# acerbilab/gpyreg

Measured on AMD Instinct MI355X. Metric: GP-fits/sec (NLL+grad, N=4096 D=10), higher is better.
Workload: dtype f64

## Files before the change

### gpyreg_amd/csrc/blas1.h

```cpp
#pragma once
#include "common.h"

namespace gpc {

template <typename T>
__global__ __launch_bounds__(256) void trmv_kernel(const T* __restrict__ W_all, long long sW, int ldw,
                                                   const double* __restrict__ r_all, int npad,
                                                   double* __restrict__ z_all, int row0) {
  using vec_t = typename MM<T>::vec_t;
  constexpr int VEC = MM<T>::VEC;
  const int b = blockIdx.y, lane = threadIdx.x & 63;
  const int i = row0 + blockIdx.x * 4 + (threadIdx.x >> 6);
  const T* Wr = W_all + (size_t)b * sW + (size_t)i * ldw;
  const double* r = r_all + (size_t)b * npad;
  const int kend = ((i >> 7) + 1) << 7;
  double s = 0.0;
  for (int k = row0 + lane * VEC; k < kend; k += 64 * VEC) {
    const vec_t wv = *reinterpret_cast<const vec_t*>(Wr + k);
#pragma unroll
    for (int e = 0; e < VEC; ++e) s += (double)wv[e] * r[k + e];
  }
  s = wave_sum(s);
  if (lane == 0) z_all[(size_t)b * npad + i] = s;
}
// ... 129 lines not shown
  __shared__ double red[4][64 * MM<T>::VEC];
  trmv_t_part_body<T, UNR>(W_all, sW, ldw, z_all, npad, part_all, quad, red);
}
template <typename T>
__global__ __launch_bounds__(256) void trmv_t_part_low_kernel(
    const T* __restrict__ W_all, long long sW, int ldw, const double* __restrict__ z_all, int npad,
    double* __restrict__ part_all, double* __restrict__ quad) {
  __shared__ double red[4][64 * MM<T>::VEC];
  __builtin_amdgcn_s_setprio(3);
  trmv_t_part_body<T, 3>(W_all, sW, ldw, z_all, npad, part_all, quad, red);
}

__global__ __launch_bounds__(128) void trmv_t_sum_kernel(const double* __restrict__ part_all, int npad,
                                                         const double* __restrict__ sp_all, int sp_stride,
                                                         int sp_off, double* __restrict__ out_all) {
  const int b = blockIdx.y, k = blockIdx.x * 128 + threadIdx.x;
  const int nch = npad / TRC;
  double v = 0.0;
  for (int ch = k / TRC; ch < nch; ++ch) v += part_all[((size_t)b * nch + ch) * npad + k];
  if (sp_all) v /= sp_all[(size_t)b * sp_stride + sp_off];
  out_all[(size_t)b * npad + k] = v;
}

__global__ __launch_bounds__(256) void dot_kernel(const double* __restrict__ x, const double* __restrict__ y,
                                                  int n, int stride, double* __restrict__ out) {
  __shared__ double sh4[4];
  const int b = blockIdx.y;
  double s = 0.0;
  for (int i = threadIdx.x; i < n; i += 256) s += x[(size_t)b * stride + i] * y[(size_t)b * stride + i];
  s = block_sum_256(s, sh4);
  if (threadIdx.x == 0) out[b] = s;
}

__global__ __launch_bounds__(256) void mat_t_vec_kernel(const double* __restrict__ Mat, int n, int P,
                                                        const double* __restrict__ vec, int vstride,
                                                        double* __restrict__ out) {
  __shared__ double sh4[4];
  const int p = blockIdx.x, b = blockIdx.y;
  double s = 0.0;
  for (int i = threadIdx.x; i < n; i += 256)
    s += Mat[((size_t)b * n + i) * P + p] * vec[(size_t)b * vstride + i];
  s = block_sum_256(s, sh4);
  if (threadIdx.x == 0) out[(size_t)b * P + p] = s;
}

__global__ __launch_bounds__(256) void grad_tail_kernel(const double* __restrict__ part, int ntiles, int P,
// ... 290 lines not shown
```

### gpyreg_amd/csrc/gemm.h

```cpp
#pragma once
#include "common.h"

#include <type_traits>

namespace gpc {

template <typename T>
constexpr int BKT_v = sizeof(T) == 4 ? 32 : 16;
template <typename T>
constexpr bool MM_SWZ = sizeof(T) == 4;
template <typename T>
constexpr int LDQ_v = MM_SWZ<T> ? BKT_v<T> : BKT_v<T> + 1;
constexpr int ldp_of(int BT) { return BT + 16; }
template <typename T>
constexpr int opsz_of(int BT) {
  return BKT_v<T> * (BT + 16) > BT * LDQ_v<T> ? BKT_v<T> * (BT + 16) : BT * LDQ_v<T>;
}

enum { KLO_ZERO = 0, KLO_ROW = 1, KLO_COL = 2 };
enum { KHI_FULL = 0, KHI_ROW = 1, KHI_COL = 2 };

struct GemmArgs {
  const void* A;
  const void* B;
  void* C;
  long long sA, sB, sC;
  int lda, ldb, ldc;
  int M, N, K;
  double alpha;
  int beta;
  int klo, khi, lower_only;
  int tiles_m, tiles_n;
  int flags = 0;
  const unsigned short* rsv = nullptr;
  int* ctr = nullptr;
  int ntiles = 0, batch = 0;
  double* colsq = nullptr;
  const double* ep_w = nullptr;
  long long ep_sw = 0;
  const double* ep_alpha = nullptr;
};
inline int g_gemm_flags = 8 | 16;

template <typename T, bool KM, int BT, int NT>
__device__ __forceinline__ unsigned stage_toff(int ld, int t) {
  constexpr int VEC = MM<T>::VEC;
  if constexpr (!KM) {
    constexpr int TPR = BKT_v<T> / VEC;
    return (unsigned)(t / TPR) * (unsigned)ld + (unsigned)((t % TPR) * VEC);
  } else {
    constexpr int VPR = BT / VEC;
    return (unsigned)(t / VPR) * (unsigned)ld + (unsigned)((t % VPR) * VEC);
  }
}
template <typename T, bool KM, int BT, int NT>
__device__ __forceinline__ size_t stage_pstride(int ld) {
  constexpr int VEC = MM<T>::VEC;
  if constexpr (!KM)
    return (size_t)(NT / (BKT_v<T> / VEC)) * ld;
  else
    return (size_t)(NT / (BT / VEC)) * ld;
}
template <typename T, bool KM, int BT, int NT, int AUX = 0>
// ... 47 lines not shown

template <typename T, bool KM, int BT>
__device__ __forceinline__ T frag(const T* __restrict__ s, int r0, int kk, int lane) {
  if constexpr (!KM) {
    if constexpr (MM_SWZ<T>) {
      constexpr int VEC = MM<T>::VEC;
      const int k = kk + (lane >> 4), l15 = lane & 15;
      return s[(r0 + l15) * LDQ_v<T> + (((k / VEC) ^ ((l15 >> 1) & 7)) * VEC) + (k % VEC)];
    } else {
      return s[(r0 + (lane & 15)) * LDQ_v<T> + kk + (lane >> 4)];
    }
  }
  else
    return s[(kk + (lane >> 4)) * ldp_of(BT) + r0 + (lane & 15)];
}

__device__ __forceinline__ void tri_tile(int tile, int& ti, int& tj) {
  int i = (int)((sqrtf(8.f * (float)tile + 1.f) - 1.f) * 0.5f);
  while (i * (i + 1) / 2 > tile) --i;
  while ((i + 1) * (i + 2) / 2 <= tile) ++i;
  ti = i;
  tj = tile - i * (i + 1) / 2;
}

#ifdef GPC_TILE_TRACE
__device__ unsigned long long g_tile_trace[2][4];
#define TILE_TS(k) do { if (HO && threadIdx.x == 0) { const long long _n = wall_clock64(); atomicAdd(&g_tile_trace[BT == 64][k], (unsigned long long)(_n - _ts)); _ts = _n; } } while (0)
#else
#define TILE_TS(k) do { } while (0)
#endif
template <typename T, bool AKM, bool BKM, int BT, int NW, int HO = 0, int EPI = 0, int BTN = BT>
__device__ __forceinline__ void gemm_tile(const GemmArgs& g, const int bx, const int by, T* __restrict__ smem) {
#ifdef GPC_TILE_TRACE
  long long _ts = wall_clock64();
  if (HO && threadIdx.x == 0) atomicAdd(&g_tile_trace[BT == 64][3], 1ull);
#endif
  using acc_t = typename MM<T>::acc_t;
  using vec_t = typename MM<T>::vec_t;
  constexpr int NT = 64 * NW;
  constexpr int NVA = (BT * BKT_v<T>) / (NT * MM<T>::VEC), NVB = (BTN * BKT_v<T>) / (NT * MM<T>::VEC);
  constexpr int OPSZA = opsz_of<T>(BT), OPSZB = opsz_of<T>(BTN), STG = OPSZA + OPSZB;
  constexpr int WCOLS = NW / 2;
  constexpr int WTM = BT / 2;
  constexpr int WTN = BTN / WCOLS;
  constexpr int MRM = WTM / 16, MRN = WTN / 16;
  static_assert(NVA >= 1 && NVB >= 1 && MRM >= 1 && MRN >= 1, "tile shape");
// ... 30 lines not shown
  int k0 = g.klo == KLO_ROW ? m128 : (g.klo == KLO_COL ? n128 : 0);
  int k1 = g.khi == KHI_ROW ? m128 + TILE : (g.khi == KHI_COL ? n128 + TILE : g.K);
  if (k1 > g.K) k1 = g.K;
  const int nk = (k1 - k0) / BKT_v<T>;

  const T* __restrict__ A = reinterpret_cast<const T*>(g.A) + (size_t)by * g.sA;
  const T* __restrict__ B = reinterpret_cast<const T*>(g.B) + (size_t)by * g.sB;
  T* __restrict__ C = reinterpret_cast<T*>(g.C) + (size_t)by * g.sC;

  acc_t acc[MRM][MRN];
#pragma unroll
  for (int i = 0; i < MRM; ++i)
#pragma unroll
    for (int j = 0; j < MRN; ++j) acc[i][j] = acc_t{0, 0, 0, 0};
  constexpr bool TWO_LEVEL = sizeof(T) == 4;
  acc_t acc2[TWO_LEVEL ? MRM : 1][TWO_LEVEL ? MRN : 1];
  if constexpr (TWO_LEVEL) {
#pragma unroll
    for (int i = 0; i < MRM; ++i)
#pragma unroll
      for (int j = 0; j < MRN; ++j) acc2[i][j] = acc_t{0, 0, 0, 0};
  }

  if (nk > 0) {
    vec_t ra[NVA], rb[NVB];
    const unsigned toa = stage_toff<T, AKM, BT, NT>(g.lda, t) * (unsigned)sizeof(T),
                   tob = stage_toff<T, BKM, BTN, NT>(g.ldb, t) * (unsigned)sizeof(T);
    const unsigned psa = (unsigned)(stage_pstride<T, AKM, BT, NT>(g.lda) * sizeof(T)),
                   psb = (unsigned)(stage_pstride<T, BKM, BTN, NT>(g.ldb) * sizeof(T));
    const T* pa = AKM ? A + (size_t)k0 * g.lda + m0 : A + (size_t)m0 * g.lda + k0;
    const T* pb = BKM ? B + (size_t)k0 * g.ldb + n0 : B + (size_t)n0 * g.ldb + k0;
    const size_t rowsa = (size_t)BKT_v<T> * g.lda, rowsb = (size_t)BKT_v<T> * g.ldb;
    __amdgpu_buffer_rsrc_t rsa = make_rsrc(pa), rsb = make_rsrc(pb);
    unsigned ua = 0, ub = 0;
    auto next_slab = [&]() {
      if constexpr (AKM) {
        pa += rowsa;
        rsa = make_rsrc(pa);
      } else {
        ua += (unsigned)(BKT_v<T> * sizeof(T));
      }
      if constexpr (BKM) {
        pb += rowsb;
        rsb = make_rsrc(pb);
      } else {
        ub += (unsigned)(BKT_v<T> * sizeof(T));
      }
    };
    constexpr int AUX = HO == 1 ? 16 : 0;
    g2r<T, AKM, BT, NT, AUX>(ra, rsa, ua, psa, toa);
    g2r<T, BKM, BTN, NT, AUX>(rb, rsb, ub, psb, tob);
    r2s<T, AKM, BT, NT>(smem, ra, t);
    r2s<T, BKM, BTN, NT>(smem + OPSZA, rb, t);
    next_slab();
    g2r<T, AKM, BT, NT, AUX>(ra, rsa, ua, psa, toa);
    g2r<T, BKM, BTN, NT, AUX>(rb, rsb, ub, psb, tob);
    __syncthreads();
    TILE_TS(0);

    T af[2][MRM], bf[2][MRN];
    auto load_frags = [&](int set, const T* a_s, const T* b_s, int kk) {
#pragma unroll
      for (int i = 0; i < MRM; ++i) af[set][i] = frag<T, AKM, BT>(a_s, wr * WTM + i * 16, kk, lane);
#pragma unroll
      for (int j = 0; j < MRN; ++j) bf[set][j] = frag<T, BKM, BTN>(b_s, wc * WTN + j * 16, kk, lane);
    };
    auto mfmas = [&](int set) {
#pragma unroll
      for (int i = 0; i < MRM; ++i)
#pragma unroll
        for (int j = 0; j < MRN; ++j) acc[i][j] = MM<T>::mma(af[set][i], bf[set][j], acc[i][j]);
    };
    constexpr int NMEM = NVA + NVB;
    constexpr int PER = (MRM * MRN) / NMEM;
    constexpr int REM = MRM * MRN - PER * NMEM;
    static_assert(PER >= 1, "interleave pattern");
    constexpr int KS = BKT_v<T> / 4;
    static_assert(KS >= 4 && KS % 2 == 0, "fragment sets alternate per k-step and wrap per slab");
    auto slab = [&](auto cur_c, auto wr_c, auto ld_c) {
// ... 124 lines not shown
          else
            v = al * acc[i][j][r];
          v += old[j][r];
          const double d = (double)v;
          cs[j] = fma(wr4[r] * d, d, cs[j]);
        }
    }
#pragma unroll
    for (int j = 0; j < MRN; ++j) {
      cs[j] += __shfl_xor(cs[j], 16, 64);
      cs[j] += __shfl_xor(cs[j], 32, 64);
    }
    double* red = reinterpret_cast<double*>(smem);
    __syncthreads();
    if ((lane >> 4) == 0) {
#pragma unroll
      for (int j = 0; j < MRN; ++j) red[wr * BT + wc * WTN + j * 16 + (lane & 15)] = cs[j];
    }
    __syncthreads();
    if (t < BT) g.colsq[((size_t)by * g.tiles_m + ti) * (size_t)g.N + n0 + t] = red[t] + red[BT + t];
    __syncthreads();
    return;
  }
#pragma unroll
  for (int i = 0; i < MRM; ++i) {
    T old[MRN][4];
    if (g.beta) {
#pragma unroll
      for (int j = 0; j < MRN; ++j)
#pragma unroll
        for (int r = 0; r < 4; ++r) {
          const int row = m0 + wr * WTM + i * 16 + MM<T>::row_of(lane, r);
          const int col = n0 + wc * WTN + j * 16 + (lane & 15);
          if constexpr (HO == 1)
            old[j][r] = __hip_atomic_load(&C[(size_t)row * g.ldc + col], __ATOMIC_RELAXED, __HIP_MEMORY_SCOPE_AGENT);
          else
            old[j][r] = C[(size_t)row * g.ldc + col];
        }
    }
#pragma unroll
    for (int j = 0; j < MRN; ++j)
#pragma unroll
      for (int r = 0; r < 4; ++r) {
        const int row = m0 + wr * WTM + i * 16 + MM<T>::row_of(lane, r);
        const int col = n0 + wc * WTN + j * 16 + (lane & 15);
        T v;
        if constexpr (TWO_LEVEL)
          v = alpha * (acc[i][j][r] + acc2[i][j][r]);
        else
          v = alpha * acc[i][j][r];
        if (g.beta) v += old[j][r];
        if constexpr (HO)
          __hip_atomic_store(&C[(size_t)row * g.ldc + col], v, __ATOMIC_RELAXED, __HIP_MEMORY_SCOPE_AGENT);
        else
          C[(size_t)row * g.ldc + col] = v;
      }
  }
  TILE_TS(2);
}

template <typename T, bool AKM, bool BKM, int BT, int NW, int EPI = 0, int BTN = BT>
__global__ __launch_bounds__(64 * NW, NW / 2) void gemm_kernel(GemmArgs g) {
  __shared__ __attribute__((aligned(16))) T smem[2 * (opsz_of<T>(BT) + opsz_of<T>(BTN))];
  int bx = blockIdx.x, by = blockIdx.y;
  if ((g.flags & 16) && gridDim.y >= 8) {
    const int total = gridDim.x * gridDim.y, per = total >> 3;
    const int L = blockIdx.y * gridDim.x + blockIdx.x;
    if (L < (per << 3)) {
      const int wk = (L & 7) * per + (L >> 3);
      bx = wk % (int)gridDim.x;
      by = wk / (int)gridDim.x;
    }
  }
  gemm_tile<T, AKM, BKM, BT, NW, 0, EPI, BTN>(g, bx, by, smem);
}

template <typename T, bool A1, bool B1, bool A2, bool B2, int BT, int NW>
__global__ __launch_bounds__(64 * NW, NW / 2) void gemm_dual_kernel(GemmArgs g1, GemmArgs g2, int n1) {
  __shared__ __attribute__((aligned(16))) T smem[4 * opsz_of<T>(BT)];
  int bx = blockIdx.x, by = blockIdx.y;
  if ((g1.flags & 16) && gridDim.y >= 8) {
// ... 59 lines not shown
}

inline int g_persist_spare = 0;
inline long long g_gemm_launches = 0;
inline int g_block_slots = 512;
template <typename T, int BT, int NW>
inline hipError_t launch_gemm_bt(hipStream_t st, GemmArgs g, bool akm, bool bkm, int batch, int* ctr = nullptr,
                                 const unsigned short* reserve = nullptr) {
  const int tm = g.M / BT, tn = g.N / BT;
  g.tiles_m = tm;
  g.tiles_n = tn;
  g.flags = g_gemm_flags;
  const int ntiles = g.lower_only ? tm * (tm + 1) / 2 : tm * tn;
  if (ntiles <= 0 || batch <= 0) return hipSuccess;
  ++g_gemm_launches;
  g.ntiles = ntiles;
  g.batch = batch;
  g.ctr = ctr;
  const unsigned dyn = 0u;
  const int cap = (BT == 128 ? g_block_slots : 2 * g_block_slots) - g_persist_spare;
  g.rsv = reserve;
  if (ctr && (BT == 128 || reserve) && cap > 0 && ((long long)ntiles * batch > cap || reserve)) {
    dim3 grid(reserve ? (BT == 128 ? cap + 96 : cap) : cap), block(64 * NW);
    if (!akm && !bkm)
      hipLaunchKernelGGL((gemm_persist_kernel<T, false, false, BT, NW>), grid, block, dyn, st, g);
    else if (!akm && bkm)
      hipLaunchKernelGGL((gemm_persist_kernel<T, false, true, BT, NW>), grid, block, dyn, st, g);
    else if (akm && bkm)
      hipLaunchKernelGGL((gemm_persist_kernel<T, true, true, BT, NW>), grid, block, dyn, st, g);
    else
      hipLaunchKernelGGL((gemm_persist_kernel<T, true, false, BT, NW>), grid, block, dyn, st, g);
    return hipGetLastError();
  }
  dim3 grid(ntiles, batch), block(64 * NW);
  if (!akm && !bkm)
    hipLaunchKernelGGL((gemm_kernel<T, false, false, BT, NW>), grid, block, dyn, st, g);
  else if (!akm && bkm)
    hipLaunchKernelGGL((gemm_kernel<T, false, true, BT, NW>), grid, block, dyn, st, g);
  else if (akm && bkm)
    hipLaunchKernelGGL((gemm_kernel<T, true, true, BT, NW>), grid, block, dyn, st, g);
  else
    hipLaunchKernelGGL((gemm_kernel<T, true, false, BT, NW>), grid, block, dyn, st, g);
  return hipGetLastError();
}

#ifdef GPC_EXPERIMENTS
template <typename T>
inline hipError_t launch_gemm_rect(hipStream_t st, GemmArgs g, bool akm, bool bkm, int batch) {
  constexpr int BT = 128, BTN = 64;
  g.tiles_m = g.M / BT;
  g.tiles_n = g.N / BTN;
  g.flags = g_gemm_flags;
  const int ntiles = g.lower_only ? g.tiles_m * (g.tiles_m + 1) : g.tiles_m * g.tiles_n;
  if (ntiles <= 0 || batch <= 0) return hipSuccess;
  ++g_gemm_launches;
  g.ntiles = ntiles;
  g.batch = batch;
  g.ctr = nullptr;
// ... 143 lines not shown
```

### gpyreg_amd/csrc/gpcore.hip

```cpp
#include "../../include/gpcore.h"

#include <algorithm>
#include <atomic>
#include <chrono>
#include <cmath>
#include <cstdlib>
#include <cstring>
#include <memory>
#include <mutex>

#include "blas1.h"
#include "block_append.h"
#include "common.h"
#include "covfun.h"
#include "cv.h"
#include "draw.h"
#include "gemm.h"
#include "leaf.h"
#include "lookahead.h"
#include "paths.h"
#include "plan.h"
#include "quad.h"
#include "quad_mix.h"
#ifdef GPC_EXPERIMENTS
// ... 343 lines not shown
    blks.clear();
    pend.clear();
  }
};

}

struct gpc_ctx {
  int device = 0;
  hipStream_t st = nullptr;
  hipEvent_t ev[4] = {nullptr, nullptr, nullptr, nullptr};
  static constexpr int MAXG = 8;
  hipStream_t gst[MAXG] = {};
  hipStream_t sst[MAXG + 1] = {};
  static constexpr int NDEV = 64;
  hipEvent_t dev_ev[MAXG + 1][NDEV] = {};
  hipEvent_t ev_bfork[MAXG + 1] = {}, ev_btail[MAXG + 1] = {};
  int defer_min = -1, defer_reserve = 8;
  unsigned cu_seen[64] = {};
  bool cu_map_ok = false;
  DevBuf rsv_tbl;
  int nll_block = -1;
  int solves_beside_lauum = 1;
#ifdef GPC_EXPERIMENTS
  int rl_panel = 0;
  int rl_ahead_max = 8;
#endif
  int stable = 0;
  int small_path = 1;
  int small_poll = 1, small_timing = 0;
  double* land_blk = nullptr;
  static constexpr size_t LAND_BYTES = 64u << 10;
  unsigned long long land_seq = 0;
  unsigned long long small_polled = 0, small_synced = 0;
  unsigned long long cov_fused = 0;
  unsigned long long quad_mix_gemms = 0;
  int check_queues = 0;
  hipEvent_t ev_up = nullptr, ev_done[MAXG] = {};
  int groups = 2;
  hipEvent_t ev_l0[MAXG + 1] = {}, ev_l1[MAXG + 1] = {};
  double ms_lauum = 0, flops_lauum = 0;
  int lauum_groups = 0;
  std::string err;
  std::string devinfo;
  int N = 0, D = 0, npad = 0;
  DevBuf dX;
  DevBuf dY;
  std::vector<double> hy;
  DevBuf mA, mW, mT;
  DevBuf xs, spb, mulb, divb;
  DevBuf dvec, rvec, zvec, avec;
  DevBuf tpart;
  DevBuf scal;
  DevBuf parts, gout, diagq;
  DevBuf dmb, dsn2b, mg, ng;
  DevBuf ks, vb, kss, xss, pout;
  DevBuf qb, gpart, gres;
  DevBuf qcon;
  DevBuf qmix;
  DevBuf zb, fb, dout, daux;
  DevBuf dbg1, dbg2, dbg3;
  PinBuf pin;
  struct GraphEntry {
    unsigned long long key[4] = {0, 0, 0, 0};
    unsigned long long epoch = 0;
    hipGraphExec_t exec = nullptr;
    unsigned long long last_use = 0;
    double flops = 0;
  };
  static constexpr int NGRAPH = 16;
  GraphEntry graphs[NGRAPH];
  unsigned long long graph_clock = 0;
  int graph_max_npad = 4096;
  bool capturing = false;
  DevBuf tile_ctr;
// ... 527 lines not shown
        F.forward_solve_nll(0, npad, rvec, zvec);
      else
        F.forward_solve(0, npad, full_inv, rvec, zvec);
      F.st = keep;
      F.low_regs = false;
      if (mode == MODE_NLL) {
        hipLaunchKernelGGL(dot_kernel, dim3(1, n), dim3(256), 0, sx, (const double*)zvec, (const double*)zvec,
                           npad, npad, d_quad);
      } else {
        double* tpart = c->tpart.as<double>() + (size_t)off * (npad / TRC) * npad;
        const dim3 gt((npad + 64 * MM<T>::VEC - 1) / (64 * MM<T>::VEC), npad / TRC, n);
        if (sx != st)
          hipLaunchKernelGGL((trmv_t_part_low_kernel<T>), gt, dim3(256), 0, sx, (const T*)Wc, sM, npad, (const double*)zvec,
                             npad, tpart, d_quad);
        else
          hipLaunchKernelGGL((trmv_t_part_kernel<T, 8>), gt, dim3(256), 0, sx, (const T*)Wc, sM, npad, (const double*)zvec,
                             npad, tpart, d_quad);
        hipLaunchKernelGGL(trmv_t_sum_kernel, dim3(npad / 128, n), dim3(128), 0, sx, (const double*)tpart, npad,
                           (const double*)spb, (int)SP_STRIDE, (int)SP_SL, avec);
      }
      HIPCHK(c, hipGetLastError());
      return 0;
    };
    hipEvent_t ev_solved = nullptr;
    if (mode == MODE_GRAD) {
      if (solves_beside_lauum) {
        hipStream_t sx = c->sst[gidx];
        hipEvent_t ev_fork = c->dev_ev[gidx][gpc_ctx::NDEV - 1];
        ev_solved = c->dev_ev[gidx][gpc_ctx::NDEV - 2];
        HIPCHK(c, hipEventRecord(ev_fork, st));
        HIPCHK(c, hipStreamWaitEvent(sx, ev_fork, 0));
        if (int rc = solves(sx)) return rc;
        HIPCHK(c, hipEventRecord(ev_solved, sx));
      }
      if (!dag_has_lauum) {
        if (!c->capturing) HIPCHK(c, hipEventRecord(c->ev_l0[gidx], st));
        F.lauum(Tc, sM);
        if (!c->capturing) {
          HIPCHK(c, hipEventRecord(c->ev_l1[gidx], st));
          lauum_n[gidx] = n;
        }
      }
    }
    HIPCHK(c, F.err);
    HIPCHK(c, hipGetLastError());
    if (f1 && !c->capturing) HIPCHK(c, hipEventRecord(f1, st));
    c->last_flops += F.flops;

    if (ev_solved)
      HIPCHK(c, hipStreamWaitEvent(st, ev_solved, 0));
    else if (int rc = solves(st))
      return rc;
    HIPCHK(c, hipGetLastError());

    const int Pn = P();
    if (mode == MODE_GRAD) {
      double* parts = c->parts.as<double>() + (size_t)off * ntl * Pn;
      double* diagq = c->diagq.as<double>() + (size_t)off * npad;
      if (kmode()) {
        hipLaunchKernelGGL((diagq_kernel<T>), dim3(1, n), dim3(256), 0, st, (const T*)Tc, sM, npad, (const double*)avec,
                           (const double*)spb, N, diagq, c->gout.as<double>() + (size_t)off * Pn, Pn);
      } else {
        GPC_COV_DISPATCH(trace_kernel, T, b.cd, dim3(ntl, n), dim3(256), 4 * (((Pn + 3) & ~3) + 4) * sizeof(double), st,
                         b.cd, (const double*)xs, (const double*)spb, (const double*)avec, N, npad, (const T*)Tc, sM,
                         npad, parts, ntl, diagq);
        const int mN = mean_N > 0 ? mean_N : 0, nN = (noise_N > 0 && b.vec_noise) ? noise_N : 0;
        hipLaunchKernelGGL(grad_tail_kernel, dim3(Pn + mN + nN, n), dim3(256), 0, st, (const double*)parts, ntl, Pn,
                           c->gout.as<double>() + (size_t)off * Pn,
                           (mN && dm) ? (const double*)(c->dmb.as<double>() + (size_t)off * N * mean_N) : nullptr, N, mN,
                           (const double*)avec, mN ? c->mg.as<double>() + (size_t)off * mean_N : nullptr,
                           nN ? (const double*)(c->dsn2b.as<double>() + (size_t)off * N * noise_N) : nullptr, nN,
                           (const double*)diagq, nN ? c->ng.as<double>() + (size_t)off * noise_N : nullptr, npad);
// ... 172 lines not shown
    }
    HIPCHK(c, hipEventRecord(ev_join, sd));
    const int nl = std::max(1, std::min(c->dag_leaf_blocks > 0 ? c->dag_leaf_blocks : std::min(n, 8), 8));
    if (c->dag_leaf_blocks >= 0)
      hipLaunchKernelGGL((dag_leaf_kernel<T>), dim3(nl), dim3(256), 0, st, d, gpc::g_leaf_fault);
    HIPCHK(c, hipStreamWaitEvent(st, ev_join, 0));
    HIPCHK(c, hipGetLastError());
    F.flops += flops1 * n;
    F.launches += 2;
    has_lauum = with_lauum;
    c->dag_used = true;
    ++c->dag_runs;
    return 0;
  }
#else
  static constexpr bool use_dag = false, indep_mode = false, use_rl = false;
#endif
  int graph_section(int cnt) {
    Batch& b = *B;
    hipStream_t st = c->st;
    const unsigned long long key[4] = {
        ((unsigned long long)mode << 60) | ((unsigned long long)sizeof(T) << 52) | ((unsigned long long)b.vec_noise << 48) |
            ((unsigned long long)prescaled << 49) | ((unsigned long long)(stable || c->stable) << 50) |
            ((unsigned long long)cnt << 24) | (unsigned long long)b.N,
        ((unsigned long long)b.cd.kind << 48) | ((unsigned long long)b.cd.degree << 40) | ((unsigned long long)b.D << 20) |
            ((unsigned long long)mean_N << 10) | (unsigned long long)noise_N,
        (unsigned long long)(uintptr_t)A, (unsigned long long)(uintptr_t)W ^ ((unsigned long long)(uintptr_t)Tm << 1)};
    gpc_ctx::GraphEntry* hit = nullptr;
    gpc_ctx::GraphEntry* victim = &c->graphs[0];
    for (auto& g : c->graphs) {
      if (g.exec && g.epoch == g_alloc_epoch && g.key[0] == key[0] && g.key[1] == key[1] && g.key[2] == key[2] &&
          g.key[3] == key[3])
        hit = &g;
      if (g.last_use < victim->last_use) victim = &g;
    }
    if (!hit) {
      if (victim->exec) {
        (void)hipGraphExecDestroy(victim->exec);
        victim->exec = nullptr;
      }
      hipGraph_t graph = nullptr;
      const double flops_before = c->last_flops;
      HIPCHK(c, hipStreamBeginCapture(st, hipStreamCaptureModeThreadLocal));
      c->capturing = true;
      const int rc = device_section(st, 0, cnt, nullptr, nullptr);
      c->capturing = false;
// ... 222 lines not shown
    chunk_cnt = cnt;
    chunk_s0 = s0;
    T* A0 = A;
    T* W0 = W;
    T* T0 = Tm;
    A = A0 + (size_t)slot * sM;
    W = W0 + (size_t)slot * sM;
    Tm = T0 + (size_t)slot * sM;
    struct Restore {
      Pipe* p;
      T *a, *w, *t;
      ~Restore() { p->A = a; p->W = w; p->Tm = t; }
    } restore{this, A0, W0, T0};

    HIPCHK(c, c->xs.ensure((size_t)cnt * npad * D * sizeof(double)));
    HIPCHK(c, c->spb.ensure((size_t)cnt * SP_STRIDE * sizeof(double)));
    HIPCHK(c, c->mulb.ensure((size_t)cnt * D * sizeof(double)));
    HIPCHK(c, c->divb.ensure((size_t)cnt * D * sizeof(double)));
    HIPCHK(c, c->dvec.ensure(cnt * vb));
    HIPCHK(c, c->rvec.ensure(cnt * vb));
    HIPCHK(c, c->zvec.ensure(cnt * vb));
    HIPCHK(c, c->avec.ensure(cnt * vb));
    HIPCHK(c, c->tpart.ensure((size_t)cnt * (npad / TRC + 1) * vb));
    HIPCHK(c, c->scal.ensure((size_t)cnt * (2 * sizeof(double) + sizeof(int)) + 64));
    double* d_logdet = c->scal.as<double>();
    double* d_quad = d_logdet + cnt;
    int* d_info = reinterpret_cast<int*>(d_quad + cnt);
    if (mode == MODE_GRAD) {
      HIPCHK(c, c->parts.ensure((size_t)cnt * ntl * Pn * sizeof(double)));
      HIPCHK(c, c->gout.ensure((size_t)cnt * Pn * sizeof(double)));
      HIPCHK(c, c->diagq.ensure(cnt * vb));
      if (mean_N > 0) {
        if (dm) HIPCHK(c, c->dmb.ensure((size_t)cnt * N * mean_N * 8));
        HIPCHK(c, c->mg.ensure((size_t)cnt * mean_N * 8));
      }
      if (noise_N > 0 && b.vec_noise) {
        HIPCHK(c, c->dsn2b.ensure((size_t)cnt * N * noise_N * 8));
        HIPCHK(c, c->ng.ensure((size_t)cnt * noise_N * 8));
      }
    }

    HostClock hc("run");
    c->pin.begin();
    c->pin.begin_gather();
    auto up = [&](void* dst, const void* src, size_t n) { return c->pin.stage(dst, src, n); };
    const bool small_cand = c->small_path && npad == TILE && !kmode() && !(stable || c->stable) && gpc::g_leaf_version == 5;
// ... 2803 lines not shown
  if (const char* e = getenv("GPC_SMALL_PATH")) c->small_path = atoi(e) != 0;
  if (const char* e = getenv("GPC_GRAPH_MAX_NPAD")) c->graph_max_npad = atoi(e);
#ifdef GPC_EXPERIMENTS
  if (const char* e = getenv("GPC_RL_PANEL")) c->rl_panel = atoi(e) <= 0 ? 0 : std::max(TILE, (atoi(e) / TILE) * TILE);
  if (const char* e = getenv("GPC_RECT_MIN")) gpc::g_rect_min_blocks = atoi(e);
#endif
  if (const char* e = getenv("GPC_NLL_BLOCK")) c->nll_block = atoi(e) < 0 ? -1 : (atoi(e) == 0 ? 0 : std::max(TILE, (atoi(e) / TILE) * TILE));
  if (const char* e = getenv("GPC_GROUPS")) c->groups = std::max(1, std::min((int)gpc_ctx::MAXG, atoi(e)));
  if (const char* e = getenv("GPC_SMALL_BLOCKS")) gpc::g_small_launch_blocks = atoi(e);
  if (const char* e = getenv("GPC_DUAL")) gpc::g_dual_launch = atoi(e) != 0;
  if (const char* e = getenv("GPC_GEMM_FLAGS")) gpc::g_gemm_flags = atoi(e);
  if (const char* e = getenv("GPC_XCD_AFFINE")) gpc::g_gemm_flags = atoi(e) ? (gpc::g_gemm_flags | 8) : (gpc::g_gemm_flags & ~8);
  *out = c;
  return 0;
}

void gpc_destroy(gpc_ctx* c) {
  if (!c) return;
  (void)hipSetDevice(c->device);
  (void)hipStreamSynchronize(c->st);
  DevBuf* bufs[] = {&c->dX,   &c->dY,  &c->mA,    &c->mW,  &c->mT,   &c->xs,   &c->spb,  &c->mulb, &c->divb,
                    &c->dvec, &c->rvec,  &c->zvec, &c->avec, &c->scal, &c->parts, &c->gout, &c->diagq,
                    &c->dmb,  &c->dsn2b, &c->mg,  &c->ng,   &c->ks,   &c->vb,   &c->xss,  &c->pout, &c->kss,
                    &c->dbg1, &c->dbg2,  &c->dbg3, &c->tpart, &c->qb, &c->gpart, &c->gres, &c->qcon, &c->qmix, &c->zb, &c->fb, &c->dout, &c->daux, &c->tile_ctr, &c->rsv_tbl};
  for (auto& g : c->graphs)
    if (g.exec) (void)hipGraphExecDestroy(g.exec);
  for (DevBuf* b : bufs) b->release();
  c->pool_drain();
  c->pin.release();
  if (c->land_blk) (void)hipHostFree(c->land_blk);
  for (auto& ev : c->ev)
    if (ev) (void)hipEventDestroy(ev);
  if (c->ev_up) (void)hipEventDestroy(c->ev_up);
  for (int g = 0; g <= gpc_ctx::MAXG; ++g) {
    if (c->ev_l0[g]) (void)hipEventDestroy(c->ev_l0[g]);
    if (c->ev_l1[g]) (void)hipEventDestroy(c->ev_l1[g]);
  }
  for (int g = 0; g <= gpc_ctx::MAXG; ++g) {
    for (int i = 0; i < gpc_ctx::NDEV; ++i)
      if (c->dev_ev[g][i]) (void)hipEventDestroy(c->dev_ev[g][i]);
    if (c->ev_bfork[g]) (void)hipEventDestroy(c->ev_bfork[g]);
    if (c->ev_btail[g]) (void)hipEventDestroy(c->ev_btail[g]);
    if (c->sst[g]) (void)hipStreamDestroy(c->sst[g]);
  }
  for (int g = 0; g < gpc_ctx::MAXG; ++g) {
    if (c->ev_done[g]) (void)hipEventDestroy(c->ev_done[g]);
    if (c->gst[g]) (void)hipStreamDestroy(c->gst[g]);
// ... 732 lines not shown
  int (*set)(gpc_ctx*, int);
};
#ifdef GPC_EXPERIMENTS
constexpr int IS_EXPERIMENTS_BUILD = 1;
#else
constexpr int IS_EXPERIMENTS_BUILD = 0;
#endif
int clamp_to(int lo, int hi, int v) { return std::max(lo, std::min(hi, v)); }
int tile_multiple(int v) { return std::max(TILE, (v / TILE) * TILE); }
int engine_choice(int v) { return v == 1 || v == 2 ? v : 0; }
#define GPC_GET(expr) [](gpc_ctx* c) -> int { (void)c; return (int)(expr); }
#define GPC_SET(stmt) [](gpc_ctx* c, int v) -> int { (void)c; stmt; return 0; }
#define GPC_COUNTER(field) GPC_GET(c->field & 0x7fffffff), nullptr
const Option OPTIONS[] = {
    {"groups", GPC_GET(c->groups), GPC_SET(c->groups = clamp_to(1, gpc_ctx::MAXG, v))},
    {"small_blocks", GPC_GET(gpc::g_small_launch_blocks), GPC_SET(gpc::g_small_launch_blocks = v)},
    {"dual_launch", GPC_GET(gpc::g_dual_launch ? 1 : 0), GPC_SET(gpc::g_dual_launch = v != 0)},
    {"leaf", GPC_GET(gpc::g_leaf_version), GPC_SET(gpc::g_leaf_version = v == 3 ? 3 : 5)},
    {"defer_min", GPC_GET(c->defer_min), GPC_SET(c->defer_min = v)},
    {"defer_reserve", GPC_GET(c->defer_reserve), [](gpc_ctx* c, int v) -> int { return c->defer_reserve = v, build_reserve_table(c); }},
    {"leaf_fault", nullptr, GPC_SET(gpc::g_leaf_fault = v != 0)},
    {"nll_block", GPC_GET(c->nll_block), GPC_SET(c->nll_block = v < 0 ? -1 : (v == 0 ? 0 : tile_multiple(v)))},
    {"solves_beside_lauum", GPC_GET(c->solves_beside_lauum), GPC_SET(c->solves_beside_lauum = v != 0)},
    {"stable", GPC_GET(c->stable), GPC_SET(c->stable = v != 0)},
    {"small_path", GPC_GET(c->small_path), GPC_SET(c->small_path = v != 0)},
    {"check_queues", GPC_GET(c->check_queues), GPC_SET(c->check_queues = v != 0)},
    {"small_poll", GPC_GET(c->small_poll), GPC_SET(c->small_poll = v != 0)},
    {"small_timing", GPC_GET(c->small_timing), GPC_SET(c->small_timing = v != 0)},
    {"small_polled", GPC_COUNTER(small_polled)},
    {"small_synced", GPC_COUNTER(small_synced)},
    {"cov_fused", GPC_COUNTER(cov_fused)},
    {"quad_mix_gemms", GPC_COUNTER(quad_mix_gemms)},
    {"start_mult_log10", nullptr, GPC_SET(c->start_mult = std::pow(10.0, clamp_to(0, 9, v)))},
    {"append_fail_mask", nullptr, GPC_SET(c->append_fail_mask = (unsigned)v)},
    {"block_engine", GPC_GET(c->block_engine), GPC_SET(c->block_engine = engine_choice(v))},
    {"block_engine_ran", GPC_GET(c->block_engine_ran), nullptr},
    {"paths_engine", GPC_GET(c->paths_engine), GPC_SET(c->paths_engine = engine_choice(v))},
    {"paths_engine_ran", GPC_GET(c->paths_engine_ran), nullptr},
    {"paths_solve_engine", GPC_GET(c->paths_solve_engine), GPC_SET(c->paths_solve_engine = engine_choice(v))},
    {"paths_solve_engine_ran", GPC_GET(c->paths_solve_engine_ran), nullptr},
    {"cv_engine", GPC_GET(c->cv_engine), GPC_SET(c->cv_engine = engine_choice(v))},
    {"cv_engine_ran", GPC_GET(c->cv_engine_ran), nullptr},
    {"block_appended", GPC_COUNTER(block_appended)},
    {"block_stale", GPC_COUNTER(block_stale)},
    {"experiments", GPC_GET(IS_EXPERIMENTS_BUILD), nullptr},
};
// ... 278 lines not shown
```

### gpyreg_amd/csrc/plan.h

```cpp
#pragma once
#include "blas1.h"
#include "gemm.h"
#include "leaf.h"

#include <algorithm>

namespace gpc {

#ifdef GPC_EXPERIMENTS
struct PlanRecorder {
  struct Op {
    int kind;
    GemmArgs g;
    bool akm, bkm;
    int off;
  };
  std::vector<Op> ops;
  bool unsupported = false;
};
#endif

template <typename T>
struct Factor {
#ifdef GPC_EXPERIMENTS
// ... 52 lines not shown
    GemmArgs g;
    g.A = Aop;
    g.B = Bop;
    g.C = C;
    g.sA = sAop;
    g.sB = sBop;
    g.sC = sC;
    g.lda = g.ldb = g.ldc = npad;
    g.M = M;
    g.N = N;
    g.K = K;
    g.alpha = alpha;
    g.beta = beta;
    g.klo = klo;
    g.khi = khi;
    g.lower_only = lower;
    g.tiles_n = N / TILE;
    flops += gemm_flops(g, batch);
    return g;
  }

  void gemm(T* C, long long sC, const T* Aop, long long sAop, const T* Bop, long long sBop, int M,
            int N, int K, bool akm, bool bkm, double alpha, int beta, int klo, int khi, int lower,
            hipStream_t on = nullptr, const unsigned short* rsv = nullptr) {
    GemmArgs g;
    g.A = Aop;
    g.B = Bop;
    g.C = C;
    g.sA = sAop;
    g.sB = sBop;
    g.sC = sC;
    g.lda = g.ldb = g.ldc = npad;
    g.M = M;
    g.N = N;
    g.K = K;
    g.alpha = alpha;
    g.beta = beta;
    g.klo = klo;
    g.khi = khi;
    g.lower_only = lower;
    g.tiles_n = N / TILE;
    flops += gemm_flops(g, batch);
    ++launches;
#ifdef GPC_EXPERIMENTS
    if (rec) {
      rec->ops.push_back({0, g, akm, bkm, 0});
      return;
    }
// ... 214 lines not shown
#endif

  bool low_regs = false;
  void forward_solve(int off, int n, bool need_inv, double* r, double* z) {
    if (need_inv || n == TILE) {
      if (low_regs && off == 0 && n == npad)
        hipLaunchKernelGGL((trmv_low_kernel<T>), dim3(n / 16, batch), dim3(256), 0, st, (const T*)W, sW, npad,
                           (const double*)r, npad, z);
      else
        hipLaunchKernelGGL((trmv_kernel<T>), dim3(n / 4, batch), dim3(256), 0, st, (const T*)W, sW, npad,
                           (const double*)r, npad, z, off);
      ++launches;
      return;
    }
    const int q = n / TILE;
    const int n1 = (q / 2) * TILE, n2 = n - n1;
    forward_solve(off, n1, true, r, z);
    hipLaunchKernelGGL((gemv_sub_kernel<T>), dim3(n2 / 4, batch), dim3(256), 0, st, (const T*)Tm, sT, npad,
                       (const double*)z, r, npad, off + n1, off, n1);
    ++launches;
    forward_solve(off + n1, n2, need_inv, r, z);
  }

  void lauum(T* out, long long sOut) {
    gemm(out, sOut, W, sW, W, sW, npad, npad, npad, true, true, 1.0, 0, KLO_ROW, KHI_FULL, 1);
  }
};

}
```

Baseline: 850.4.

## Fuse alpha = K^-1 r computation into LAUUM GEMM epilogue

Adds a GEMM epilogue to the lauum (W^T W = K^-1) kernel that multiplies each output tile by r and writes row and column partial sums per 64-chunk. A new alpha_reduce_kernel then sums these partials into alpha and computes the quadratic term r·alpha, using an atomic last-block reduction. This replaces the separate triangular solves (trmv and transpose) on the gradient path, along with the side-stream fork and join. In exchange, the lauum epilogue gets heavier, the partial buffers take extra memory, and the summation order changes slightly.

Measured after the change: 856.1 (median of 6 runs). No clear change (+0.7%).

```diff
diff --git a/gpyreg_amd/csrc/blas1.h b/gpyreg_amd/csrc/blas1.h
--- a/gpyreg_amd/csrc/blas1.h
+++ b/gpyreg_amd/csrc/blas1.h
@@ -175,6 +175,47 @@
   out_all[(size_t)b * npad + k] = v;
 }
 
+__global__ __launch_bounds__(128) void alpha_reduce_kernel(const double* __restrict__ prow_all,
+                                                           const double* __restrict__ pcol_all, int npad,
+                                                           const double* __restrict__ r_all,
+                                                           const double* __restrict__ sp_all, int sp_stride, int sp_off,
+                                                           double* __restrict__ alpha_all, double* __restrict__ quad,
+                                                           double* __restrict__ qpart_all, unsigned* __restrict__ ctr) {
+#pragma clang fp contract(off)
+  __shared__ double sh2[2];
+  const int b = blockIdx.y, i = blockIdx.x * 128 + threadIdx.x;
+  const int nch = npad >> 6, ci = i >> 6, nblk = gridDim.x;
+  const double* prow = prow_all + (size_t)b * nch * npad + i;
+  const double* pcol = pcol_all + (size_t)b * nch * npad + i;
+  double v = 0.0;
+  for (int c0 = 0; c0 < nch; c0 += 16) {
+    double p[16];
+#pragma unroll
+    for (int u = 0; u < 16; ++u) {
+      const int ch = c0 + u;
+      p[u] = ch < nch ? (ch <= ci ? prow : pcol)[(size_t)ch * npad] : 0.0;
+    }
+#pragma unroll
+    for (int u = 0; u < 16; ++u)
+      if (c0 + u < nch) v += p[u];
+  }
+  alpha_all[(size_t)b * npad + i] = v / sp_all[(size_t)b * sp_stride + sp_off];
+  const double q = wave_sum(r_all[(size_t)b * npad + i] * v);
+  if ((threadIdx.x & 63) == 0) sh2[threadIdx.x >> 6] = q;
+  __syncthreads();
+  if (threadIdx.x == 0) {
+    double* qpart = qpart_all + (size_t)b * nblk;
+    __hip_atomic_store(qpart + blockIdx.x, sh2[0] + sh2[1], __ATOMIC_RELAXED, __HIP_MEMORY_SCOPE_AGENT);
+    const unsigned before = __hip_atomic_fetch_add(ctr + b, 1u, __ATOMIC_ACQ_REL, __HIP_MEMORY_SCOPE_AGENT);
+    if (before == (unsigned)nblk - 1u) {
+      double s = 0.0;
+      for (int k = 0; k < nblk; ++k) s += __hip_atomic_load(qpart + k, __ATOMIC_RELAXED, __HIP_MEMORY_SCOPE_AGENT);
+      quad[b] = s;
+      __hip_atomic_store(ctr + b, 0u, __ATOMIC_RELAXED, __HIP_MEMORY_SCOPE_AGENT);
+    }
+  }
+}
+
 __global__ __launch_bounds__(256) void dot_kernel(const double* __restrict__ x, const double* __restrict__ y,
                                                   int n, int stride, double* __restrict__ out) {
   __shared__ double sh4[4];
diff --git a/gpyreg_amd/csrc/gemm.h b/gpyreg_amd/csrc/gemm.h
--- a/gpyreg_amd/csrc/gemm.h
+++ b/gpyreg_amd/csrc/gemm.h
@@ -39,6 +39,7 @@
   const double* ep_w = nullptr;
   long long ep_sw = 0;
   const double* ep_alpha = nullptr;
+  double* colsq2 = nullptr;
 };
 inline int g_gemm_flags = 8 | 16;
 
@@ -132,6 +133,40 @@
   ti = i;
   tj = tile - i * (i + 1) / 2;
 }
+
+template <int NV>
+__device__ __forceinline__ double lane16_sums(double (&x)[NV], int lane) {
+#pragma clang fp contract(off)
+  static_assert(NV == 8 || NV == 16, "eight or sixteen values per lane");
+  int n = NV;
+#pragma unroll
+  for (int m = 1; m < 16; m <<= 1) {
+    if (n > 1) {
+      const bool hi = (lane & m) != 0;
+#pragma unroll
+      for (int p = 0; p < n / 2; ++p) {
+        const double keep = hi ? x[2 * p + 1] : x[2 * p], send = hi ? x[2 * p] : x[2 * p + 1];
+        x[p] = keep + __shfl_xor(send, m, 64);
+      }
+      n /= 2;
+    } else {
+      x[0] += __shfl_xor(x[0], m, 64);
+    }
+  }
+  return x[0];
+}
+
+template <bool ON, int N>
+struct EpiShared {
+  static __device__ __forceinline__ double* get() {
+    __shared__ double a[N];
+    return a;
+  }
+};
+template <int N>
+struct EpiShared<false, N> {
+  static __device__ __forceinline__ double* get() { return nullptr; }
+};
 
 #ifdef GPC_TILE_TRACE
 __device__ unsigned long long g_tile_trace[2][4];
@@ -208,7 +243,14 @@
       for (int j = 0; j < MRN; ++j) acc2[i][j] = acc_t{0, 0, 0, 0};
   }
 
+  constexpr bool R_LDS = EPI == 3 && BT == 128;
+  double* const r_sh = EpiShared<R_LDS, 2 * BT>::get();
   if (nk > 0) {
+    double r_mine = 0.0;
+    if constexpr (R_LDS) {
+      static_assert(!R_LDS || NT == 2 * BT, "one element of r per thread");
+      r_mine = (g.ep_w + (size_t)by * (size_t)g.N)[t < BT ? m0 + t : n0 + t - BT];
+    }
     vec_t ra[NVA], rb[NVB];
     const unsigned toa = stage_toff<T, AKM, BT, NT>(g.lda, t) * (unsigned)sizeof(T),
                    tob = stage_toff<T, BKM, BTN, NT>(g.ldb, t) * (unsigned)sizeof(T);
@@ -241,6 +283,7 @@
     next_slab();
     g2r<T, AKM, BT, NT, AUX>(ra, rsa, ua, psa, toa);
     g2r<T, BKM, BTN, NT, AUX>(rb, rsb, ub, psb, tob);
+    if constexpr (R_LDS) r_sh[t] = r_mine;
     __syncthreads();
     TILE_TS(0);
 
@@ -411,6 +454,21 @@
     __syncthreads();
     return;
   }
+  [[maybe_unused]] int te = t;
+  [[maybe_unused]] double rc_g[MRN], rr_g[MRM][4];
+  if constexpr (EPI == 3) {
+    asm volatile("" : "+v"(te));
+    if constexpr (!R_LDS) {
+      const double* __restrict__ rv = g.ep_w + (size_t)by * (size_t)g.N;
+      const int ew = te >> 6;
+#pragma unroll
+      for (int j = 0; j < MRN; ++j) rc_g[j] = rv[n0 + (ew % WCOLS) * WTN + j * 16 + (te & 15)];
+#pragma unroll
+      for (int i = 0; i < MRM; ++i)
+#pragma unroll
+        for (int r = 0; r < 4; ++r) rr_g[i][r] = rv[m0 + (ew / WCOLS) * WTM + i * 16 + MM<T>::row_of(te & 63, r)];
+    }
+  }
 #pragma unroll
   for (int i = 0; i < MRM; ++i) {
     T old[MRN][4];
@@ -446,6 +504,108 @@
       }
   }
   TILE_TS(2);
+  if constexpr (EPI == 3) {
+#pragma clang fp contract(off)
+    static_assert(NW == 4 && BTN == BT && (BT == 128 || BT == 64) && HO == 0, "2 x 2 waves of 64 x 64 or 32 x 32");
+    const int ln = te & 63, q = te & 15, ew = te >> 6, er = ew / WCOLS, ec = ew % WCOLS;
+    const int nch = g.N >> 6;
+    const int bi = (m0 >> 6) + (BT == 128 ? er : 0), bj = (n0 >> 6) + (BT == 128 ? ec : 0);
+    const bool rows_on = bi >= bj, cols_on = bi > bj;
+    const int rbase = m0 + er * WTM, cbase = n0 + ec * WTN;
+    auto val = [&](int i, int j, int r) -> double {
+      if constexpr (TWO_LEVEL)
+        return (double)(T)(alpha * (acc[i][j][r] + acc2[i][j][r]));
+      else
+        return (double)(T)(alpha * acc[i][j][r]);
+    };
+    constexpr int LG = MRN == 4 ? 2 : 1;
+    static_assert(MRN == (1 << LG) && MRM == MRN, "fragments per wave");
+    double rowp[MRM], colp[MRN];
+    if (rows_on) {
+      double rc[MRN];
+#pragma unroll
+      for (int j = 0; j < MRN; ++j) {
+        if constexpr (R_LDS)
+          rc[j] = r_sh[BT + ec * WTN + j * 16 + q];
+        else
+          rc[j] = rc_g[j];
+      }
+#pragma unroll
+      for (int i = 0; i < MRM; ++i) {
+        double x[4 * MRN];
+#pragma unroll
+        for (int r = 0; r < 4; ++r)
+#pragma unroll
+          for (int j = 0; j < MRN; ++j) x[r * MRN + j] = val(i, j, r) * rc[j];
+        double s = lane16_sums<4 * MRN>(x, ln);
+#pragma unroll
+        for (int m = 1; m < MRN; m <<= 1) s += __shfl_xor(s, m, 64);
+        rowp[i] = s;
+      }
+    }
+    if (cols_on) {
+      double pr[MRM / 2][MRN];
+#pragma unroll
+      for (int i = 0; i < MRM; ++i) {
+        double rr[4];
+#pragma unroll
+        for (int r = 0; r < 4; ++r) {
+          if constexpr (R_LDS)
+            rr[r] = r_sh[er * WTM + i * 16 + MM<T>::row_of(ln, r)];
+          else
+            rr[r] = rr_g[i][r];
+        }
+#pragma unroll
+        for (int j = 0; j < MRN; ++j) {
+          double s = 0.0;
+#pragma unroll
+          for (int r = 0; r < 4; ++r) s = fma(val(i, j, r), rr[r], s);
+          s += __shfl_xor(s, 16, 64);
+          s += __shfl_xor(s, 32, 64);
+          if (i & 1)
+            pr[i / 2][j] += s;
+          else
+            pr[i / 2][j] = s;
+        }
+      }
+#pragma unroll
+      for (int j = 0; j < MRN; ++j) {
+        if constexpr (MRM == 4)
+          colp[j] = pr[0][j] + pr[1][j];
+        else
+          colp[j] = pr[0][j];
+      }
+    }
+    double* __restrict__ prow = g.colsq + ((size_t)by * nch + bj) * (size_t)g.N;
+    double* __restrict__ pcol = g.colsq2 + ((size_t)by * nch + bi) * (size_t)g.N;
+    if constexpr (BT == 128) {
+      if (rows_on && (q & (MRN - 1)) == 0) {
+#pragma unroll
+        for (int i = 0; i < MRM; ++i) prow[rbase + i * 16 + MM<T>::row_of(ln, q >> LG)] = rowp[i];
+      }
+      if (cols_on && ln < 16) {
+#pragma unroll
+        for (int j = 0; j < MRN; ++j) pcol[cbase + j * 16 + q] = colp[j];
+      }
+    } else {
+      double* red = reinterpret_cast<double*>(smem);
+      __syncthreads();
+      if (q < 8 && (q & (MRN - 1)) == 0) {
+#pragma unroll
+        for (int i = 0; i < MRM; ++i) red[ec * 64 + er * WTM + i * 16 + MM<T>::row_of(ln, q >> LG)] = rowp[i];
+      }
+      if (cols_on && ln < 16) {
+#pragma unroll
+        for (int j = 0; j < MRN; ++j) red[128 + er * 64 + ec * WTN + j * 16 + q] = colp[j];
+      }
+      __syncthreads();
+      if (te < 64)
+        prow[m0 + te] = red[te] + red[64 + te];
+      else if (te < 128 && cols_on)
+        pcol[n0 + te - 64] = red[128 + te - 64] + red[192 + te - 64];
+      __syncthreads();
+    }
+  }
 }
 
 template <typename T, bool AKM, bool BKM, int BT, int NW, int EPI = 0, int BTN = BT>
@@ -551,7 +711,9 @@
   g.rsv = reserve;
   if (ctr && (BT == 128 || reserve) && cap > 0 && ((long long)ntiles * batch > cap || reserve)) {
     dim3 grid(reserve ? (BT == 128 ? cap + 96 : cap) : cap), block(64 * NW);
-    if (!akm && !bkm)
+    if (g.colsq2)
+      hipLaunchKernelGGL((gemm_persist_kernel<T, true, true, BT, NW, 3>), grid, block, dyn, st, g);
+    else if (!akm && !bkm)
       hipLaunchKernelGGL((gemm_persist_kernel<T, false, false, BT, NW>), grid, block, dyn, st, g);
     else if (!akm && bkm)
       hipLaunchKernelGGL((gemm_persist_kernel<T, false, true, BT, NW>), grid, block, dyn, st, g);
@@ -562,7 +724,9 @@
     return hipGetLastError();
   }
   dim3 grid(ntiles, batch), block(64 * NW);
-  if (!akm && !bkm)
+  if (g.colsq2)
+    hipLaunchKernelGGL((gemm_kernel<T, true, true, BT, NW, 3>), grid, block, dyn, st, g);
+  else if (!akm && !bkm)
     hipLaunchKernelGGL((gemm_kernel<T, false, false, BT, NW>), grid, block, dyn, st, g);
   else if (!akm && bkm)
     hipLaunchKernelGGL((gemm_kernel<T, false, true, BT, NW>), grid, block, dyn, st, g);
diff --git a/gpyreg_amd/csrc/gpcore.hip b/gpyreg_amd/csrc/gpcore.hip
--- a/gpyreg_amd/csrc/gpcore.hip
+++ b/gpyreg_amd/csrc/gpcore.hip
@@ -389,6 +389,7 @@
   DevBuf rsv_tbl;
   int nll_block = -1;
   int solves_beside_lauum = 1;
+  int alpha_epilogue = 1;
 #ifdef GPC_EXPERIMENTS
   int rl_panel = 0;
   int rl_ahead_max = 8;
@@ -418,6 +419,7 @@
   DevBuf xs, spb, mulb, divb;
   DevBuf dvec, rvec, zvec, avec;
   DevBuf tpart;
+  DevBuf epart, eaux, ectr;
   DevBuf scal;
   DevBuf parts, gout, diagq;
   DevBuf dmb, dsn2b, mg, ng;
@@ -991,9 +993,10 @@
       HIPCHK(c, hipGetLastError());
       return 0;
     };
+    const bool alpha_epi = mode == MODE_GRAD && c->alpha_epilogue && !kmode() && !dag_has_lauum && npad > TILE;
     hipEvent_t ev_solved = nullptr;
     if (mode == MODE_GRAD) {
-      if (solves_beside_lauum) {
+      if (solves_beside_lauum && !alpha_epi) {
         hipStream_t sx = c->sst[gidx];
         hipEvent_t ev_fork = c->dev_ev[gidx][gpc_ctx::NDEV - 1];
         ev_solved = c->dev_ev[gidx][gpc_ctx::NDEV - 2];
@@ -1004,11 +1007,20 @@
       }
       if (!dag_has_lauum) {
         if (!c->capturing) HIPCHK(c, hipEventRecord(c->ev_l0[gidx], st));
-        F.lauum(Tc, sM);
+        double* ep = c->epart.as<double>() + (size_t)off * 2 * (npad / 64) * npad;
+        if (alpha_epi)
+          F.lauum(Tc, sM, rvec, ep, ep + (size_t)n * (npad / 64) * npad);
+        else
+          F.lauum(Tc, sM);
         if (!c->capturing) {
           HIPCHK(c, hipEventRecord(c->ev_l1[gidx], st));
           lauum_n[gidx] = n;
         }
+        if (alpha_epi)
+          hipLaunchKernelGGL(alpha_reduce_kernel, dim3(npad / 128, n), dim3(128), 0, st, (const double*)ep,
+                             (const double*)(ep + (size_t)n * (npad / 64) * npad), npad, (const double*)rvec,
+                             (const double*)spb, (int)SP_STRIDE, (int)SP_SL, avec, d_quad,
+                             c->eaux.as<double>() + (size_t)off * (npad / 128), c->ectr.as<unsigned>() + off);
       }
     }
     HIPCHK(c, F.err);
@@ -1016,7 +1028,8 @@
     if (f1 && !c->capturing) HIPCHK(c, hipEventRecord(f1, st));
     c->last_flops += F.flops;
 
-    if (ev_solved)
+    if (alpha_epi) {
+    } else if (ev_solved)
       HIPCHK(c, hipStreamWaitEvent(st, ev_solved, 0));
     else if (int rc = solves(st))
       return rc;
@@ -1235,6 +1248,7 @@
     const unsigned long long key[4] = {
         ((unsigned long long)mode << 60) | ((unsigned long long)sizeof(T) << 52) | ((unsigned long long)b.vec_noise << 48) |
             ((unsigned long long)prescaled << 49) | ((unsigned long long)(stable || c->stable) << 50) |
+            ((unsigned long long)(c->alpha_epilogue != 0) << 51) |
             ((unsigned long long)cnt << 24) | (unsigned long long)b.N,
         ((unsigned long long)b.cd.kind << 48) | ((unsigned long long)b.cd.degree << 40) | ((unsigned long long)b.D << 20) |
             ((unsigned long long)mean_N << 10) | (unsigned long long)noise_N,
@@ -1503,6 +1517,15 @@
     HIPCHK(c, c->zvec.ensure(cnt * vb));
     HIPCHK(c, c->avec.ensure(cnt * vb));
     HIPCHK(c, c->tpart.ensure((size_t)cnt * (npad / TRC + 1) * vb));
+    if (mode == MODE_GRAD && c->alpha_epilogue && !kmode() && npad > TILE) {
+      HIPCHK(c, c->epart.ensure((size_t)cnt * 2 * (npad / 64) * vb));
+      HIPCHK(c, c->eaux.ensure((size_t)cnt * (npad / 128) * sizeof(double)));
+      if (c->ectr.bytes < (size_t)cnt * sizeof(unsigned)) {
+        HIPCHK(c, c->ectr.ensure((size_t)cnt * sizeof(unsigned) + 256));
+        HIPCHK(c, hipMemsetAsync(c->ectr.p, 0, c->ectr.bytes, st));
+        HIPCHK(c, hipStreamSynchronize(st));
+      }
+    }
     HIPCHK(c, c->scal.ensure((size_t)cnt * (2 * sizeof(double) + sizeof(int)) + 64));
     double* d_logdet = c->scal.as<double>();
     double* d_quad = d_logdet + cnt;
@@ -4352,7 +4375,7 @@
   DevBuf* bufs[] = {&c->dX,   &c->dY,  &c->mA,    &c->mW,  &c->mT,   &c->xs,   &c->spb,  &c->mulb, &c->divb,
                     &c->dvec, &c->rvec,  &c->zvec, &c->avec, &c->scal, &c->parts, &c->gout, &c->diagq,
                     &c->dmb,  &c->dsn2b, &c->mg,  &c->ng,   &c->ks,   &c->vb,   &c->xss,  &c->pout, &c->kss,
-                    &c->dbg1, &c->dbg2,  &c->dbg3, &c->tpart, &c->qb, &c->gpart, &c->gres, &c->qcon, &c->qmix, &c->zb, &c->fb, &c->dout, &c->daux, &c->tile_ctr, &c->rsv_tbl};
+                    &c->dbg1, &c->dbg2,  &c->dbg3, &c->tpart, &c->epart, &c->eaux, &c->ectr, &c->qb, &c->gpart, &c->gres, &c->qcon, &c->qmix, &c->zb, &c->fb, &c->dout, &c->daux, &c->tile_ctr, &c->rsv_tbl};
   for (auto& g : c->graphs)
     if (g.exec) (void)hipGraphExecDestroy(g.exec);
   for (DevBuf* b : bufs) b->release();
@@ -5131,6 +5154,7 @@
     {"leaf_fault", nullptr, GPC_SET(gpc::g_leaf_fault = v != 0)},
     {"nll_block", GPC_GET(c->nll_block), GPC_SET(c->nll_block = v < 0 ? -1 : (v == 0 ? 0 : tile_multiple(v)))},
     {"solves_beside_lauum", GPC_GET(c->solves_beside_lauum), GPC_SET(c->solves_beside_lauum = v != 0)},
+    {"alpha_epilogue", GPC_GET(c->alpha_epilogue), GPC_SET(c->alpha_epilogue = v != 0)},
     {"stable", GPC_GET(c->stable), GPC_SET(c->stable = v != 0)},
     {"small_path", GPC_GET(c->small_path), GPC_SET(c->small_path = v != 0)},
     {"check_queues", GPC_GET(c->check_queues), GPC_SET(c->check_queues = v != 0)},
diff --git a/gpyreg_amd/csrc/plan.h b/gpyreg_amd/csrc/plan.h
--- a/gpyreg_amd/csrc/plan.h
+++ b/gpyreg_amd/csrc/plan.h
@@ -98,8 +98,13 @@
 
   void gemm(T* C, long long sC, const T* Aop, long long sAop, const T* Bop, long long sBop, int M,
             int N, int K, bool akm, bool bkm, double alpha, int beta, int klo, int khi, int lower,
-            hipStream_t on = nullptr, const unsigned short* rsv = nullptr) {
+            hipStream_t on = nullptr, const unsigned short* rsv = nullptr, const double* ep_r = nullptr,
+            double* ep_prow = nullptr, double* ep_pcol = nullptr) {
     GemmArgs g;
+    g.ep_w = ep_r;
+    g.ep_sw = npad;
+    g.colsq = ep_prow;
+    g.colsq2 = ep_pcol;
     g.A = Aop;
     g.B = Bop;
     g.C = C;
@@ -360,8 +365,9 @@
     forward_solve(off + n1, n2, need_inv, r, z);
   }
 
-  void lauum(T* out, long long sOut) {
-    gemm(out, sOut, W, sW, W, sW, npad, npad, npad, true, true, 1.0, 0, KLO_ROW, KHI_FULL, 1);
+  void lauum(T* out, long long sOut, const double* r = nullptr, double* prow = nullptr, double* pcol = nullptr) {
+    gemm(out, sOut, W, sW, W, sW, npad, npad, npad, true, true, 1.0, 0, KLO_ROW, KHI_FULL, 1, nullptr, nullptr, r, prow,
+         pcol);
   }
 };
 
```
